# jeff-regier/Celeste.jl

Hardware: AMD Instinct MI355X
Metric: sources/sec (ELBO value+gradient+Hessian+KL per target source) (higher is better)
Workload: dtype f64; 1 GPU; BASELINE.json configs[2]: synthetic 2048x1489x5 SDSS-size field, 2000 star+galaxy sources, fp64, Sa=1 with value-only neighbours, psf_K=2; gather_backend=none, neighbor_links_rank0=3526

## Files before the change

celeste.jl_amd/csrc/celeste_abi.hip:

```cpp
#include <hip/hip_runtime.h>
#include <algorithm>
#include <atomic>
#include <cmath>
#include <cstdio>
#include <cstdlib>
#include <cstring>
#include <mutex>
#include <unordered_map>
#include <vector>

#include "elbo_kernels.h"
#include "optim_kernels.h"
#include "fused_kernels.h"
#include "host_tables.h"
#include "value_union.h"

struct celeste_group;

#define EVAL_FUSED_MAX 32

#define HIP_TRY(expr)                                                                    \
    do {                                                                                 \
        hipError_t e__ = (expr);                                                         \
        if (e__ != hipSuccess) {                                                         \
// ... 941 lines not shown
    HIP_TRY(hipGetLastError());
    return CELESTE_OK;
}

struct celeste_targets {
    celeste_ctx_t *ctx = nullptr;
    int32_t n = 0;
    int G = 1;
    int32_t *d_targets = nullptr;
    int32_t *d_work = nullptr, *d_work_total = nullptr, *d_rec_off = nullptr;
    int2 *d_items = nullptr;
    int32_t *d_needed = nullptr;
    int32_t *d_visits = nullptr;
    int32_t *d_vitems = nullptr;
    int4 *d_uitems = nullptr;
    int32_t *d_upx = nullptr;
    int64_t n_visits = 0, n_vitems = 0, n_uitems = 0;
    int64_t n_records = 0;
    int32_t n_work = 0;
    WorkSeqDesc *d_desc = nullptr;
    int32_t n_desc = 0;
};
static const int32_t LIST_STAMP = 1;

static void targets_free(celeste_targets *t) {
    if (!t) return;
    void *ptrs[] = {t->d_targets, t->d_work, t->d_work_total, t->d_rec_off, t->d_items, t->d_needed, t->d_visits, t->d_vitems,
                    t->d_uitems, t->d_upx, t->d_desc};
    for (void *p : ptrs) if (p) (void)hipFree(p);
    delete t;
}
// ... 6 lines not shown
    t->ctx = c; t->n = n; t->G = chunk_group(n);
    int32_t *d_blk = nullptr;
    auto fail = [&](int st) { if (d_blk) (void)hipFree(d_blk); (void)hipGetLastError(); targets_free(t); return st; };
#define LIST_TRY(expr) do { if ((expr) != hipSuccess) return fail(CELESTE_ERR_HIP); } while (0)
#define LIST_ALLOC(p, bytes) do { if (hipMalloc((void **)&(p), (bytes)) != hipSuccess) return fail(CELESTE_ERR_ALLOC); } while (0)
    std::vector<char> is_tgt((size_t)c->S, 0), reads((size_t)c->S, 0);
    for (int32_t s : tg) {
        is_tgt[s] = 1; reads[s] = 1;
        for (int64_t q = c->h_nbr_off[s]; q < c->h_nbr_off[s + 1]; ++q) reads[c->h_nbr_idx[q]] = 1;
        t->n_records += c->h_src_chunks[s];
    }
    std::vector<int32_t> visits, vitems;
    for (int s = 0; s < c->S; ++s)
        if (reads[s]) for (int v = c->h_vis_off[s]; v < c->h_vis_off[s + 1]; ++v) visits.push_back(v);
    for (size_t i = 0; i < c->h_vitem_tgt.size(); ++i) if (is_tgt[c->h_vitem_tgt[i]]) vitems.push_back((int32_t)i);
    std::vector<int32_t> upx;
    std::vector<ValueUnionItem> uitems;
    {
        static_assert(sizeof(ValueUnionBox) == 4 * sizeof(int32_t) && sizeof(ValueUnionItem) == sizeof(int4), "layout");
        std::vector<ValueUnionBox> boxes(c->h_patches.size());
        for (size_t v = 0; v < boxes.size(); ++v) { const DevPatch &q = c->h_patches[v]; boxes[v] = {q.off_h, q.off_w, q.H2, q.W2}; }
        std::vector<ValueUnionLink> links;
        links.reserve(vitems.size());
        for (int32_t i : vitems) links.push_back(c->h_vitem_link[(size_t)i]);
        if (!value_union_build(boxes.data(), std::move(links), c->chunk_px, upx, uitems)) return fail(CELESTE_ERR_INVALID_ARG);
    }
    t->n_visits = (int64_t)visits.size(); t->n_vitems = (int64_t)vitems.size(); t->n_uitems = (int64_t)uitems.size();
    const int n_cand = n * c->M;
    const int n_wblk = (n_cand + WORK_NT - 1) / WORK_NT;
    const size_t n_blk = (size_t)n_wblk * (WORK_CLASSES + 1);
    LIST_ALLOC(t->d_targets, (size_t)n * sizeof(int32_t));
    LIST_ALLOC(t->d_work, std::max<size_t>((size_t)t->n_records, 1) * sizeof(int32_t));
    LIST_ALLOC(t->d_work_total, sizeof(int32_t));
    LIST_ALLOC(t->d_rec_off, (size_t)n_cand * sizeof(int32_t));
    if (!c->dense) LIST_ALLOC(t->d_items, (size_t)n_cand * sizeof(int2));
    LIST_ALLOC(t->d_needed, (size_t)c->S * sizeof(int32_t));
    LIST_ALLOC(t->d_visits, std::max<size_t>(visits.size(), 1) * sizeof(int32_t));
    LIST_ALLOC(t->d_vitems, std::max<size_t>(vitems.size(), 1) * sizeof(int32_t));
    LIST_ALLOC(t->d_uitems, std::max<size_t>(uitems.size(), 1) * sizeof(int4));
    LIST_ALLOC(t->d_upx, std::max<size_t>(upx.size(), 1) * sizeof(int32_t));
    LIST_ALLOC(d_blk, n_blk * sizeof(int32_t));
    LIST_TRY(hipMemcpy(t->d_targets, tg.data(), (size_t)n * sizeof(int32_t), hipMemcpyHostToDevice));
    if (!visits.empty()) LIST_TRY(hipMemcpy(t->d_visits, visits.data(), visits.size() * sizeof(int32_t), hipMemcpyHostToDevice));
    if (!vitems.empty()) LIST_TRY(hipMemcpy(t->d_vitems, vitems.data(), vitems.size() * sizeof(int32_t), hipMemcpyHostToDevice));
    if (!uitems.empty()) LIST_TRY(hipMemcpy(t->d_uitems, uitems.data(), uitems.size() * sizeof(int4), hipMemcpyHostToDevice));
    if (!upx.empty()) LIST_TRY(hipMemcpy(t->d_upx, upx.data(), upx.size() * sizeof(int32_t), hipMemcpyHostToDevice));
    LIST_TRY(hipMemset(t->d_needed, 0, (size_t)c->S * sizeof(int32_t)));
    const size_t setup_threads = (size_t)n * (c->dense ? 1 : c->M);
    hipLaunchKernelGGL(setup_kernel, dim3((unsigned)((setup_threads + 63) / 64)), dim3(64), 0, nullptr, (const double *)nullptr, -1,
                       (SrcGeo *)nullptr, t->d_targets, n, c->d_vis_off, c->d_vis_img, c->M, t->d_items, t->d_needed, LIST_STAMP,
                       (int32_t *)nullptr, c->d_nbr_off, c->d_nbr_idx, (const int32_t *)nullptr);
    hipLaunchKernelGGL(work_count_kernel, dim3(n_wblk), dim3(WORK_NT), 0, nullptr, t->d_targets, n_cand, c->d_patches,
                       c->d_vis_off, c->d_vis_img, c->N, c->M, c->chunk_px, t->G, (int)c->dense, d_blk, (const int32_t *)nullptr);
    hipLaunchKernelGGL(work_scan_kernel, dim3(1), dim3(1024), 0, nullptr, d_blk, (int)n_blk, t->d_work_total, n_wblk * WORK_CLASSES);
    hipLaunchKernelGGL(work_fill_kernel, dim3(n_wblk), dim3(WORK_NT), 0, nullptr, t->d_targets, n_cand, c->d_patches,
                       c->d_vis_off, c->d_vis_img, c->N, c->M, c->CH, c->chunk_px, t->G, (int)c->dense, d_blk, t->d_work,
                       (const int32_t *)nullptr, t->d_rec_off);
    LIST_TRY(hipGetLastError());
    LIST_TRY(hipMemcpy(&t->n_work, t->d_work_total, sizeof(int32_t), hipMemcpyDeviceToHost));
    LIST_TRY(hipFree(d_blk)); d_blk = nullptr;
    if (t->n_work < 0 || (int64_t)t->n_work > t->n_records) return fail(CELESTE_ERR_HIP);
// ... 85 lines not shown
    if (need > c->acc_cap) {
        if (c->d_acc) { HIP_TRY(hipStreamSynchronize(stream)); HIP_TRY(hipFree(c->d_acc)); c->d_acc = nullptr; }
        HIP_TRY(hipMalloc((void **)&c->d_acc, need * sizeof(double)));
        c->acc_cap = need;
    }
    const int CH = c->CH, chunk_px = c->chunk_px;
    if (c->timing) HIP_TRY(hipEventRecord(c->ev[0], stream));
    const unsigned geo_blocks = (unsigned)((c->S + 63) / 64);
    hipLaunchKernelGGL(geo_prep_kernel, dim3(geo_blocks + (unsigned)t->n_visits), dim3(64), 0, stream, d_vp, c->d_images,
                       c->d_patches, c->d_vis_src, c->d_vis_img, c->K, c->d_srcimg, c->d_comps, t->d_visits, (int)geo_blocks,
                       c->S, c->d_geo);
    const char *no_union = getenv("CELESTE_NO_VALUE_UNION");
    if (!(no_union && atoi(no_union) != 0)) {
        if (t->n_uitems > 0) {
            const bool wide_items = n_targets <= VALUE_WIDE_MAX && c->chunk_px == 256 && !getenv("CELESTE_NO_WIDE_VALUE");
#define LAUNCH_UNION(WAVES)                                                                                                 \
            hipLaunchKernelGGL((value_union_kernel<WAVES>), dim3((unsigned)t->n_uitems), dim3(64 * WAVES), 0, stream,       \
                               c->d_patches, c->d_coefs, c->d_srcimg, c->d_comps, c->d_val_off, t->d_uitems, t->d_upx,      \
                               c->NC, c->d_val)
            if (wide_items) LAUNCH_UNION(4); else LAUNCH_UNION(1);
#undef LAUNCH_UNION
        }
    } else if (t->n_vitems > 0) {
        const bool wide_items = n_targets <= VALUE_WIDE_MAX && c->chunk_px == 256 && !getenv("CELESTE_NO_WIDE_VALUE");
#define LAUNCH_VALUE(WAVES)                                                                                                 \
        hipLaunchKernelGGL((value_kernel<double, WAVES>), dim3((unsigned)t->n_vitems), dim3(64 * WAVES), 0, stream,        \
                           c->d_patches, c->d_coefs, c->d_srcimg, c->d_comps, t->d_needed, LIST_STAMP, c->d_val_off,        \
                           c->d_value_items, c->NC, c->chunk_px, c->d_val, c->d_coefs_f, t->d_vitems)
        if (wide_items) LAUNCH_VALUE(4); else LAUNCH_VALUE(1);
#undef LAUNCH_VALUE
    }
    if (c->timing) HIP_TRY(hipEventRecord(c->ev[1], stream));
    const char *no_seq = getenv("CELESTE_NO_SEQUENCES");
    const bool sequences = !(no_seq && atoi(no_seq) != 0);
    const dim3 grid((unsigned)std::max<int32_t>(sequences ? t->n_desc : t->n_work, 1));
// ... 1086 lines not shown
```

celeste.jl_amd/csrc/elbo_kernels.h:

```cpp
#pragma once
#include <hip/hip_runtime.h>
#include <math.h>
#include "elbo_device.h"
#include "work_sequences.h"
#include "../../include/celeste_mi355x.h"

#ifndef CELESTE_MUTANT
#define CELESTE_MUTANT 0
#endif

__constant__ double c_eta[16];
__constant__ double c_nu[16];

__device__ inline void bvn_cov(double ab, double angle, double scale, double &x11, double &x12, double &x22) {
    double sp, cp;
    sincos(angle, &sp, &cp);
    double ab_term = ab * ab - 1.0;
    double s2 = scale * scale;
    x12 = -s2 * cp * sp * ab_term;
    x11 = s2 * (1.0 + ab_term * (sp * sp));
    x22 = s2 * (1.0 + ab_term * (cp * cp));
}

__device__ inline void brightness(const double *vs, int i, int b, double &El, double &Ell) {
// ... 323 lines not shown
#endif
    p = __builtin_fma(p, r, 1.6666666666666666e-01);
    p = __builtin_fma(p, r, 0.5);
    p = __builtin_fma(p, r, 1.0);
    return __builtin_fma(p, r, 1.0);
}
__device__ __forceinline__ double exp_nonpos(double x, const double *tab) {
    const double n = rint(x * EXP_INV_STEP);
    double r = __builtin_fma(n, -EXP_STEP_HI, x);
    r = __builtin_fma(n, EXP_STEP_LO, r);
    const int ni = (int)n;
    const double tj = tab[ni & (EXP_T - 1)];
    return ldexp(exp_poly(r) * tj, ni >> EXP_TAB_LOG2);
}

__device__ __forceinline__ double rcp_pos(double b) {
    double r = __builtin_amdgcn_rcp(b);
    r = __builtin_fma(__builtin_fma(-b, r, 1.0), r, r);
    return __builtin_fma(__builtin_fma(-b, r, 1.0), r, r);
}
__device__ __forceinline__ double log_pos(double x) {
    const bool ok = x > 2.2250738585072014e-308 && x < INFINITY;
    const double bad = x == INFINITY ? x : __builtin_nan("");
    double m = __builtin_amdgcn_frexp_mant(x);
    int e = __builtin_amdgcn_frexp_exp(x);
    const bool low = m < 0.7071067811865476;
    m = low ? m + m : m; e = low ? e - 1 : e;
    const double a = m - 1.0, b = m + 1.0, r = rcp_pos(b);
    double sq = a * r;
    sq = __builtin_fma(__builtin_fma(-b, sq, a), r, sq);
    const double z = sq * sq;
    double p = 1.0 / 21.0;
    p = __builtin_fma(p, z, 1.0 / 19.0); p = __builtin_fma(p, z, 1.0 / 17.0); p = __builtin_fma(p, z, 1.0 / 15.0);
    p = __builtin_fma(p, z, 1.0 / 13.0); p = __builtin_fma(p, z, 1.0 / 11.0); p = __builtin_fma(p, z, 1.0 / 9.0);
    p = __builtin_fma(p, z, 1.0 / 7.0); p = __builtin_fma(p, z, 1.0 / 5.0); p = __builtin_fma(p, z, 1.0 / 3.0);
    const double t = sq * z * p, ef = (double)e;
    const double lg = __builtin_fma(ef, 0x1.62e42fee00000p-1, (sq + sq) + __builtin_fma(ef, 0x1.a39ef35793c76p-33, t + t));
    return ok ? lg : bad;
}

__device__ inline double star_value(const double *__restrict__ coef, double xh, double xw) {
    int ix = (int)floor(xh); ix = ix < 1 ? 1 : (ix > 50 ? 50 : ix);
    int iy = (int)floor(xw); iy = iy < 1 ? 1 : (iy > 50 ? 50 : iy);
    double wx[4], wy[4];
    bspline_w(xh - ix, wx); bspline_w(xw - iy, wy);
    const double *c0 = coef + (ix - 1) + CEL_COEF * (iy - 1);
    double y = 0;
#pragma unroll
    for (int b = 0; b < 4; ++b) {
        const double *cb = c0 + CEL_COEF * b;
        double r = cb[0] * wx[0] + cb[1] * wx[1] + cb[2] * wx[2] + cb[3] * wx[3];
        y += r * wy[b];
    }
    return y < 0 ? 1e-3 * exp(y) : 1e-3 * (y + 1.0);
}

__device__ inline double galaxy_value(const Comp *tc, int NC, double dx, double dy, const double *etab) {
    double v = 0;
    const int n_dev = 8 * (NC / 14);
    for (int c0 = 0; c0 < NC; c0 += (c0 < n_dev ? 8 : 6)) {
        const int len = c0 < n_dev ? 8 : 6;
        const double d1 = dx - tc[c0].xi1, d2 = dy - tc[c0].xi2;
        const double s11 = -0.5 * (d1 * d1), s12 = -(d1 * d2), s22 = -0.5 * (d2 * d2);
        for (int c = c0; c < c0 + len; ++c) {
            const Comp k = tc[c];
            v = __builtin_fma(k.w0, exp_nonpos(__builtin_fma(k.p11, s11, __builtin_fma(k.p12, s12, k.p22 * s22)), etab), v);
        }
    }
    return v;
}

__device__ inline float star_value_f(const double *__restrict__ coef, float xh, float xw) {
    int ix = (int)floorf(xh); ix = ix < 1 ? 1 : (ix > 50 ? 50 : ix);
    int iy = (int)floorf(xw); iy = iy < 1 ? 1 : (iy > 50 ? 50 : iy);
    float wx[4], wy[4];
    bspline_w(xh - (float)ix, wx); bspline_w(xw - (float)iy, wy);
    const double *c0 = coef + (ix - 1) + CEL_COEF * (iy - 1);
    float y = 0;
#pragma unroll
    for (int b = 0; b < 4; ++b) {
        const double *cb = c0 + CEL_COEF * b;
        const float r = (float)cb[0] * wx[0] + (float)cb[1] * wx[1] + (float)cb[2] * wx[2] + (float)cb[3] * wx[3];
        y += r * wy[b];
// ... 347 lines not shown
            int first;
            const int n_rec = describe_target_records(ti, targets[ti], patches, nullptr, N, M, fz_chunk_px, rec_off, fz_chunk_desc, first);
            fz_tgt_rec[ti] = make_int2(first < 0 ? 0 : first, n_rec);
        }
    }
}

template <bool COH, typename R = double>
__device__ __forceinline__ void value_pixel(const DevPatch &P, const SrcImg &si, const Comp *__restrict__ tc, int NC,
                                            const double *__restrict__ coef, const double *__restrict__ etab, double sh0,
                                            double sw0, int h0, int w0, double2 *__restrict__ out,
                                            const float *__restrict__ tcf = nullptr) {
    const double hh = (double)(h0 + 1), ww = (double)(w0 + 1);
    double f0, f1;
    if constexpr (sizeof(R) == 8) {
        f0 = star_value(coef, hh + sh0, ww + sw0);
        f1 = galaxy_value(tc, NC, hh - si.m1, ww - si.m2, etab);
    } else {
        f0 = (double)star_value_f(coef, (float)(hh + sh0), (float)(ww + sw0));
        f1 = (double)galaxy_value_f(tcf, NC, (float)(hh - si.m1), (float)(ww - si.m2));
    }
    const double En = si.c0 * f0 + si.c1 * f1;
    const double E2n = si.q0 * (f0 * f0) + si.q1 * (f1 * f1);
    double2 *const o = out + ((h0 - P.off_h) + (int64_t)P.H2 * (w0 - P.off_w));
    const double var = E2n - En * En;
    if constexpr (COH) { stc<true>(&o->x, En); stc<true>(&o->y, var); }
    else *o = make_double2(En, var);
}

template <bool COH, typename R = double>
__device__ __forceinline__ void value_pixels(int lane, const DevPatch &P, const SrcImg &si, const Comp *__restrict__ tc, int NC,
// ... 149 lines not shown
        value_pixels<false, R>(threadIdx.x, P, si, tc, NC, coefs, etab, h_lo, w_lo, RH, p0, p1, val + val_off[sn], tcf);
    else {
        const int q0 = p0 + 64 * (int)(threadIdx.x >> 6);
        if (q0 < p1) value_pixels<false, R>(threadIdx.x & 63, P, si, tc, NC, coefs, etab, h_lo, w_lo, RH, q0, min(p1, q0 + 64), val + val_off[sn], tcf);
    }
    VT(2);
#ifdef VALUE_TIMING
    if (threadIdx.x == 0) {
        for (int k = 0; k < 3; ++k) atomicAdd(&g_value_clk[k], (unsigned long long)(vts[k + 1] - vts[k]));
        atomicAdd(&g_value_clk[7], 1ull); atomicAdd(&g_value_clk[6], (unsigned long long)((p1 - p0 + 63) / 64));
    }
#endif
#undef VT
}

template <int WAVES = 1>
__global__ void __launch_bounds__(64 * WAVES)
value_union_kernel(const DevPatch *__restrict__ patches, const double *__restrict__ coefs,
                   const SrcImg *__restrict__ srcimg, const Comp *__restrict__ comps, const int64_t *__restrict__ val_off,
                   const int4 *__restrict__ items, const int32_t *__restrict__ px_off, int NC, double2 *__restrict__ val) {
    __shared__ double etab[64];
    const int4 it = items[blockIdx.x];
    const int sn = it.x, count = it.z;
    const int32_t *__restrict__ po = px_off + it.y;
    const int lane = threadIdx.x & 63;
    int o0 = 0, o1 = 0, o2 = 0, o3 = 0;
    if constexpr (WAVES == 1) {
        if (lane < count) o0 = po[lane];
        if (lane + 64 < count) o1 = po[lane + 64];
        if (lane + 128 < count) o2 = po[lane + 128];
        if (lane + 192 < count) o3 = po[lane + 192];
    } else if ((int)threadIdx.x < count) o0 = po[threadIdx.x];
    const DevPatch &P = patches[sn];
    exp_table_init(etab);
    const SrcImg si = srcimg[sn];
    __shared__ Comp tc[14 * CEL_MAXK];
    {
        const double *src = reinterpret_cast<const double *>(comps + (size_t)sn * NC);
        double *dst = reinterpret_cast<double *>(tc);
        for (int i = threadIdx.x; i < NC * 8; i += 64 * WAVES) dst[i] = src[i];
        __syncthreads();
    }
    const double *__restrict__ coef = coefs + (size_t)(CELESTE_MUTANT == 3 ? 0 : P.stamp) * (CEL_COEF * CEL_COEF);
    const double sh0 = 26.0 - si.m1, sw0 = 26.0 - si.m2;
    const int H2 = P.H2;
    const float rH2 = 1.0f / (float)H2;
    double2 *__restrict__ out = val + val_off[sn];
    if constexpr (WAVES == 1) {
        for (int base = 0;;) {
            const int n = min(count - base, 256);
            for (int p = lane; p < n; p += 64) {
                int cw, ch;
                divmod_small(o0, H2, rH2, cw, ch);
                o0 = o1; o1 = o2; o2 = o3;
                value_pixel<false, double>(P, si, tc, NC, coef, etab, sh0, sw0, P.off_h + ch, P.off_w + cw, out);
            }
            base += 256;
            if (base >= count) break;
            const int i = base + lane;
            o0 = i < count ? po[i] : 0; o1 = i + 64 < count ? po[i + 64] : 0;
            o2 = i + 128 < count ? po[i + 128] : 0; o3 = i + 192 < count ? po[i + 192] : 0;
        }
    } else if ((int)threadIdx.x < count) {
        int cw, ch;
        divmod_small(o0, H2, rH2, cw, ch);
        value_pixel<false, double>(P, si, tc, NC, coef, etab, sh0, sw0, P.off_h + ch, P.off_w + cw, out);
    }
}

template <typename S>
struct PixelTermsT {
    typedef S scalar;
    S vterm, cnt_act, cnt_inact;
    S f0, f1;
    S alpha, beta, w2, w12;
    S k0, k1;
    S f0g0, f0g1, f0h0, f0h1, f0h2;
    S C0s, C0g, C1s, C1g;
    S Q0s, Q0g, Q1s, Q1g;
    S Wgg, Wsg, Wss;
    S S0d, S1x, S1y, S1xd, S1yd, S2a, S2b, S2c, S2an, S2bn, S2cn, S2ad, S2bd, S2cd;
    S S3a, S3b, S3c, S3d, S4a, S4b, S4c, S4d, S4e;
// ... 487 lines not shown
        const bool in_range = base + lane < p1;
        int w2, h2;
        divmod_small(idx, H2, 1.0f / (float)H2, w2, h2);
        const int h = P.off_h + h2 + 1, w = P.off_w + w2 + 1;
        const double hh = (double)h, ww = (double)w;
#define LOAD_PIXEL_INPUTS() load_pixel_inputs<MULTI, COHV>(img, P, W.patches, W.bitmaps, W.nbr_idx, W.nv, W.nb0, W.nb1, W.val_off, \
                                                     W.val, W.active_rank, W.my_rank, W.N, W.n, H2, h, w, h2, w2, in_range)
        const bool own_geo = in_range && (w2 < W2 - 1);
        if (MODE == 0) {
            const PixelInputs I = LOAD_PIXEL_INPUTS();
            const bool valid = I.valid, dup = I.dup, own = valid && own_geo;
            const double x = I.x, Ebar = I.Ebar, Vbar = I.Vbar, lgx = I.lgx, iota = I.iota, log_iota = I.log_iota;
            const int n_inact = I.n_inact;
            double f0 = 0, f1 = 0;
            if (own) {
                f0 = star_value(tcoef, hh + sh0, ww + sw0);
                f1 = galaxy_value(W.tc, NC, hh - si.m1, ww - si.m2, etab);
            }
            if (valid) {
                const double c0 = si.c0, c1 = si.c1, q0 = si.q0, q1 = si.q1;
                const double A = c0 * f0 + c1 * f1;
                const double E = Ebar + A;
                const double V = Vbar + ((q0 * (f0 * f0) + q1 * (f1 * f1)) - A * A);
                const double iE = 1.0 / E;
                if (!(MULTI && dup)) a[0] += x * (log_iota + (log(E) - V * (0.5 * iE * iE))) - iota * E - lgx;
                a[1] += own ? 1.0 : 0.0;
                a[2] += (double)n_inact;
            }
            return;
        }

// ... 1381 lines not shown
    const SrcImg si = srcimg[sn];
    __shared__ Comp tc[14 * CEL_MAXK];
    {
        const double *src = reinterpret_cast<const double *>(comps + (size_t)sn * NC);
        double *dst = reinterpret_cast<double *>(tc);
        for (int i = threadIdx.x; i < NC * 8; i += 64) dst[i] = src[i];
        __syncthreads();
    }
    const double *__restrict__ coef = coefs + (size_t)(CELESTE_MUTANT == 3 ? 0 : P.stamp) * (CEL_COEF * CEL_COEF);
    for (int idx = p0 + (int)threadIdx.x; idx < p1; idx += 64) {
        const int w2 = idx / H2, h2 = idx - w2 * H2;
        const size_t gi = (size_t)(P.off_h + h2) + (size_t)imgH * (P.off_w + w2);
        bool act = P.bitmap_off >= 0 ? bitmaps[P.bitmap_off + h2 + (int64_t)H2 * w2] != 0 : !isnan(pixels[gi]);
        if (!act) continue;
        const double hh = (double)(P.off_h + h2 + 1), ww = (double)(P.off_w + w2 + 1);
        const double f0 = star_value(coef, hh + (26.0 - si.m1), ww + (26.0 - si.m2));
        const double f1 = galaxy_value(tc, NC, hh - si.m1, ww - si.m2, etab);
        atomicAdd(&plane[gi], si.c0 * f0 + si.c1 * f1);
    }
}

__global__ void psf_raster_kernel(const double *__restrict__ psf, int K, const double *__restrict__ rows, int nr,
                                  const double *__restrict__ cols, int nc, double *__restrict__ out) {
    const int idx = blockIdx.x * blockDim.x + threadIdx.x;
    if (idx >= nr * nc) return;
    const int c = idx / nr, r = idx - c * nr;
    double s = 0;
    for (int k = 0; k < K; ++k) {
        const double *pc = psf + 6 * k;
        const double x0 = rows[r] - pc[1], x1 = cols[c] - pc[2];
        const double det = pc[3] * pc[5] - pc[4] * pc[4];
// ... 7 lines not shown
```

celeste.jl_amd/csrc/fit/celeste_fit.hip:

```cpp
#include "../celeste_abi.hip"
#include "../../../include/celeste_fit.h"

#define FIT_NB CELESTE_FIT_BANDS
#define FIT_NS CELESTE_FIT_NSTATS
#define FIT_REC 8

struct FitItem {
    int32_t sn, n;
    int32_t p0;
    int32_t rec0;
    int64_t stamp_off;
};

struct FitTileInfo { int32_t n_pix, bad, band, pad; };

__device__ __forceinline__ double fit_light(const SrcImg &si, const Comp *tc, int NC, const double *__restrict__ coef,
                                            const double *etab, double hh, double ww) {
    const double f0 = star_value(coef, hh + (26.0 - si.m1), ww + (26.0 - si.m2));
    const double f1 = galaxy_value(tc, NC, hh - si.m1, ww - si.m2, etab);
    return si.c0 * f0 + si.c1 * f1;
}

__device__ __forceinline__ double fit_wave_max(double x) {
#pragma unroll
    for (int o = 32; o >= 1; o >>= 1) x = fmax(x, __shfl_xor(x, o, 64));
    return x;
}

__device__ __forceinline__ void fit_stage_comps(Comp *dst, const Comp *__restrict__ src, int NC) {
    const double *s = reinterpret_cast<const double *>(src);
    double *d = reinterpret_cast<double *>(dst);
    for (int i = threadIdx.x; i < NC * 8; i += 64) d[i] = s[i];
}
// ... 268 lines not shown
```

celeste.jl_amd/csrc/mcmc/celeste_mcmc.hip:

```cpp
#include <hip/hip_runtime.h>
#include <algorithm>
#include <cmath>
#include <cstdio>
#include <cstring>
#include <mutex>
#include <new>
#include <vector>

#include "../elbo_kernels.h"
#include "../host_tables.h"
#include "../../../include/celeste_mcmc.h"

#define MC_D CELESTE_MCMC_D
#define MC_STEP_OUT 10
#define MC_ACCEPT_MAX 1000
#define MC_SHRINK_DEFAULT 10000

struct U4 { uint32_t x[4]; };
__host__ __device__ inline U4 philox4x32_10(U4 c, uint32_t k0, uint32_t k1) {
    for (int r = 0; r < 10; ++r) {
        if (r) { k0 += 0x9E3779B9u; k1 += 0xBB67AE85u; }
        const uint64_t p0 = (uint64_t)0xD2511F53u * c.x[0], p1 = (uint64_t)0xCD9E8D57u * c.x[2];
        U4 o;
        o.x[0] = (uint32_t)(p1 >> 32) ^ c.x[1] ^ k0;
// ... 80 lines not shown
    const double *coef = A.coefs + (size_t)P.stamp * (CEL_COEF * CEL_COEF);
    for (int64_t e = A.nbr_off[src]; e < A.nbr_off[src + 1]; ++e) {
        const celeste_mcmc_source_t &n = A.sources[A.nbr_idx[e]];
        double vs[6] = {n.pos[0], n.pos[1], n.gal_frac_dev, n.gal_axis_ratio, n.gal_angle, n.gal_radius_px};
        double m1, m2;
        world_to_pix(vs, P, m1, m2);
        const bool star = n.is_star != 0;
        const double flux = star ? n.star_fluxes[b] : n.gal_fluxes[b];
        __syncthreads();
        if (!star) prep_visit_values<false>(lane, vs, P, b, A.K, nullptr, tc);
        __syncthreads();
        const double sh0 = 26.0 - m1, sw0 = 26.0 - m2;
        for (int idx = lane; idx < npx; idx += 64) {
            const int w2 = idx / P.H2, h2 = idx - w2 * P.H2;
            const double hh = (double)(P.off_h + h2 + 1), ww = (double)(P.off_w + w2 + 1);
            const double f = star ? star_value(coef, hh + sh0, ww + sw0) : galaxy_value(tc, A.NC, hh - m1, ww - m2, etab);
            A.bgf[po + idx] = (float)((double)A.bgf[po + idx] + f * flux);
        }
    }
    for (int idx = lane; idx < npx; idx += 64) A.bg[po + idx] = (double)A.bgf[po + idx];
}

__device__ inline void mc_position(const double *box, const double *th, double &ra, double &dec) {
    ra = (box[1] - box[0]) * th[5] + box[0];
    dec = (box[3] - box[2]) * th[6] + box[2];
}

__device__ double mc_loglike(const McArgs &A, int ti, int model, const double *th, Comp *tc, const double *etab, int lane) {
    double ra, dec;
    mc_position(A.box + 4 * ti, th, ra, dec);
    double vs[6] = {ra, dec, 0.0, 0.0, 0.0, 0.0};
// ... 7 lines not shown
        const double flux = exp(th[b]);
        if (isinf(flux)) return -INFINITY;
        double m1, m2;
        world_to_pix(vs, P, m1, m2);
        if (model == 1) {
            __syncthreads();
            prep_visit_values<false>(lane, vs, P, b, A.K, nullptr, tc);
            __syncthreads();
        }
        const double *coef = A.coefs + (size_t)P.stamp * (CEL_COEF * CEL_COEF);
        const double sh0 = 26.0 - m1, sw0 = 26.0 - m2;
        const int64_t po = A.mv_pix[v];
        for (int idx = lane; idx < npx; idx += 64) {
            const int w2 = idx / P.H2, h2 = idx - w2 * P.H2;
            const double hh = (double)(P.off_h + h2 + 1), ww = (double)(P.off_w + w2 + 1);
            const double f = model == 0 ? star_value(coef, hh + sh0, ww + sw0) : galaxy_value(tc, A.NC, hh - m1, ww - m2, etab);
            const float srcf = (float)(f * flux);
            const double rate = ((double)srcf + A.bg[po + idx]) * (double)img.iota[P.off_h + h2];
            inf |= isinf(rate);
            const double x = A.data[po + idx];
            if (!isnan(x)) acc += x * log(rate) - rate;
        }
        lgs += A.lg[v];
    }
    if (__any(inf)) return -INFINITY;
    return wave_sum(acc) - lgs;
}

__device__ inline double mc_logsumexp8(const double *x) {
    double m = x[0];
    for (int k = 1; k < 8; ++k) m = fmax(m, x[k]);
// ... 613 lines not shown
```

celeste.jl_amd/csrc/synth/celeste_synth.hip:

```cpp
#include <hip/hip_runtime.h>
#include <algorithm>
#include <cmath>
#include <cstring>
#include <mutex>
#include <vector>

#include "../elbo_kernels.h"
#include "../host_tables.h"
#include "../../../include/celeste_synth.h"
#include "synth_sampler.h"

#define SYN_TH 64
#define SYN_TW 32
#define SYN_WAVES 4
#define SYN_COLS (SYN_TW / SYN_WAVES)
#define SYN_CHUNK 64
#define SYN_NCMAX (14 * CELESTE_SYNTH_MAX_K)

struct SynImage {
    int32_t H, W, K;
    uint32_t stream;
    const float *sky;
    const float *iota;
    double *lam;
// ... 70 lines not shown
            if (stamp < 0) {
                __syncthreads();
                const double *src = reinterpret_cast<const double *>(A.tables + (size_t)ent[e].table * SYN_NCMAX);
                for (int k = threadIdx.x; k < NC * (int)(sizeof(Comp) / sizeof(double)); k += 256) reinterpret_cast<double *>(tc)[k] = src[k];
                __syncthreads();
            }
            const int h0 = ent[e].h0, h1 = ent[e].h1, w0 = ent[e].w0, w1 = ent[e].w1;
            const double m1 = ent[e].m1, m2 = ent[e].m2, flux = ent[e].flux;
            const double *coef = A.coefs + (size_t)(stamp < 0 ? 0 : stamp) * (CEL_COEF * CEL_COEF);
            if (row_ok && h >= h0 && h <= h1) {
#pragma unroll
                for (int j = 0; j < SYN_COLS; ++j) {
                    const int w = T.w_start + wv + SYN_WAVES * j + 1;
                    if (w < w0 || w > w1) continue;
                    const double ww = (double)w;
                    const double f = stamp >= 0 ? star_value(coef, hh - m1 + 26.0, ww - m2 + 26.0)
                                                : galaxy_value(tc, NC, hh - m1, ww - m2, etab);
                    acc[j] += f * flux;
                }
            }
        }
    }
    if (!row_ok) return;
    const double iota = (double)img.iota[h - 1];
    unsigned long long ncap = 0;
    for (int j = 0; j < SYN_COLS; ++j) {
        const int w = T.w_start + wv + SYN_WAVES * j + 1;
        if (w > img.W) continue;
        const size_t q = (size_t)(h - 1) + (size_t)img.H * (w - 1);
        const double lam = acc[j] * iota;
        if (img.lam) img.lam[q] = lam;
// ... 259 lines not shown
```

celeste.jl_amd/csrc/value_union.h:

```cpp
#pragma once
#include <algorithm>
#include <cstddef>
#include <cstdint>
#include <vector>

struct ValueUnionBox { int32_t off_h, off_w, H2, W2; };
struct ValueUnionLink { int32_t vb, va; };
struct ValueUnionItem { int32_t vb, first, count, trips; };

inline bool value_union_build(const ValueUnionBox *boxes, std::vector<ValueUnionLink> links, int chunk_px,
                              std::vector<int32_t> &offsets, std::vector<ValueUnionItem> &items) {
    offsets.clear(); items.clear();
    std::sort(links.begin(), links.end(), [](const ValueUnionLink &a, const ValueUnionLink &b) {
        return a.vb != b.vb ? a.vb < b.vb : a.va < b.va;
    });
    links.erase(std::unique(links.begin(), links.end(), [](const ValueUnionLink &a, const ValueUnionLink &b) {
        return a.vb == b.vb && a.va == b.va;
    }), links.end());
    const int n_cls = chunk_px / 64;
    std::vector<std::vector<ValueUnionItem>> by_len((size_t)std::max(n_cls, 1));
    std::vector<unsigned char> wanted;
    for (size_t i = 0; i < links.size();) {
        const int32_t vb = links[i].vb;
        const ValueUnionBox &b = boxes[vb];
        const size_t npx = b.H2 > 0 && b.W2 > 0 ? (size_t)b.H2 * (size_t)b.W2 : 0;
        wanted.assign(npx, 0);
        for (; i < links.size() && links[i].vb == vb; ++i) {
            const ValueUnionBox &a = boxes[links[i].va];
            const int64_t h_lo = std::max(a.off_h, b.off_h), h_hi = std::min((int64_t)a.off_h + a.H2, (int64_t)b.off_h + b.H2);
            const int64_t w_lo = std::max(a.off_w, b.off_w), w_hi = std::min((int64_t)a.off_w + a.W2, (int64_t)b.off_w + b.W2 - 1);
            for (int64_t w = w_lo; w < w_hi; ++w)
                for (int64_t h = h_lo; h < h_hi; ++h) wanted[(size_t)((h - b.off_h) + (int64_t)b.H2 * (w - b.off_w))] = 1;
        }
        const size_t first = offsets.size();
        for (size_t p = 0; p < npx; ++p) if (wanted[p]) offsets.push_back((int32_t)p);
        const size_t count = offsets.size() - first;
        if (offsets.size() > (size_t)INT32_MAX) { offsets.clear(); items.clear(); return false; }
        for (size_t p0 = 0; p0 < count; p0 += (size_t)chunk_px) {
            const int32_t px = (int32_t)std::min((size_t)chunk_px, count - p0), trips = (px + 63) / 64;
            by_len[(size_t)(n_cls - trips)].push_back({vb, (int32_t)(first + p0), px, trips});
        }
    }
    for (auto &v : by_len) items.insert(items.end(), v.begin(), v.end());
    return true;
}
```

Before: 3.243 million sources/sec.

## Precompute packed (h,w) offsets, hoist star spline weights, cheaper exp in value path

The value-union builder now emits pixel offsets packed as 16-bit row/column pairs, so the kernel no longer needs a per-pixel divmod. When every lane's sub-cell fraction matches the first pixel, the kernel hoists the star B-spline weights into wave-uniform scalars, and falls back to the old path otherwise. Galaxy exp evaluation pre-scales its arguments by the inverse step and uses an unnormalised polynomial with one final rescale. The star softplus uses a table-based degree-5 exp. These changes cut VALU work in the value-only neighbour pass, at the cost of small numeric differences and a new wave ballot per pixel.

```diff
diff --git a/celeste.jl_amd/csrc/celeste_abi.hip b/celeste.jl_amd/csrc/celeste_abi.hip
--- a/celeste.jl_amd/csrc/celeste_abi.hip
+++ b/celeste.jl_amd/csrc/celeste_abi.hip
@@ -979,7 +979,7 @@
     int32_t *d_visits = nullptr;
     int32_t *d_vitems = nullptr;
     int4 *d_uitems = nullptr;
-    int32_t *d_upx = nullptr;
+    uint32_t *d_upx = nullptr;
     int64_t n_visits = 0, n_vitems = 0, n_uitems = 0;
     int64_t n_records = 0;
     int32_t n_work = 0;
@@ -1016,7 +1016,8 @@
     for (int s = 0; s < c->S; ++s)
         if (reads[s]) for (int v = c->h_vis_off[s]; v < c->h_vis_off[s + 1]; ++v) visits.push_back(v);
     for (size_t i = 0; i < c->h_vitem_tgt.size(); ++i) if (is_tgt[c->h_vitem_tgt[i]]) vitems.push_back((int32_t)i);
-    std::vector<int32_t> upx;
+    std::vector<int32_t> uoff;
+    std::vector<uint32_t> upx;
     std::vector<ValueUnionItem> uitems;
     {
         static_assert(sizeof(ValueUnionBox) == 4 * sizeof(int32_t) && sizeof(ValueUnionItem) == sizeof(int4), "layout");
@@ -1025,7 +1026,7 @@
         std::vector<ValueUnionLink> links;
         links.reserve(vitems.size());
         for (int32_t i : vitems) links.push_back(c->h_vitem_link[(size_t)i]);
-        if (!value_union_build(boxes.data(), std::move(links), c->chunk_px, upx, uitems)) return fail(CELESTE_ERR_INVALID_ARG);
+        if (!value_union_build(boxes.data(), std::move(links), c->chunk_px, uoff, uitems, &upx)) return fail(CELESTE_ERR_INVALID_ARG);
     }
     t->n_visits = (int64_t)visits.size(); t->n_vitems = (int64_t)vitems.size(); t->n_uitems = (int64_t)uitems.size();
     const int n_cand = n * c->M;
@@ -1040,13 +1041,13 @@
     LIST_ALLOC(t->d_visits, std::max<size_t>(visits.size(), 1) * sizeof(int32_t));
     LIST_ALLOC(t->d_vitems, std::max<size_t>(vitems.size(), 1) * sizeof(int32_t));
     LIST_ALLOC(t->d_uitems, std::max<size_t>(uitems.size(), 1) * sizeof(int4));
-    LIST_ALLOC(t->d_upx, std::max<size_t>(upx.size(), 1) * sizeof(int32_t));
+    LIST_ALLOC(t->d_upx, std::max<size_t>(upx.size(), 1) * sizeof(uint32_t));
     LIST_ALLOC(d_blk, n_blk * sizeof(int32_t));
     LIST_TRY(hipMemcpy(t->d_targets, tg.data(), (size_t)n * sizeof(int32_t), hipMemcpyHostToDevice));
     if (!visits.empty()) LIST_TRY(hipMemcpy(t->d_visits, visits.data(), visits.size() * sizeof(int32_t), hipMemcpyHostToDevice));
     if (!vitems.empty()) LIST_TRY(hipMemcpy(t->d_vitems, vitems.data(), vitems.size() * sizeof(int32_t), hipMemcpyHostToDevice));
     if (!uitems.empty()) LIST_TRY(hipMemcpy(t->d_uitems, uitems.data(), uitems.size() * sizeof(int4), hipMemcpyHostToDevice));
-    if (!upx.empty()) LIST_TRY(hipMemcpy(t->d_upx, upx.data(), upx.size() * sizeof(int32_t), hipMemcpyHostToDevice));
+    if (!upx.empty()) LIST_TRY(hipMemcpy(t->d_upx, upx.data(), upx.size() * sizeof(uint32_t), hipMemcpyHostToDevice));
     LIST_TRY(hipMemset(t->d_needed, 0, (size_t)c->S * sizeof(int32_t)));
     const size_t setup_threads = (size_t)n * (c->dense ? 1 : c->M);
     hipLaunchKernelGGL(setup_kernel, dim3((unsigned)((setup_threads + 63) / 64)), dim3(64), 0, nullptr, (const double *)nullptr, -1,
@@ -1162,11 +1163,15 @@
     if (!(no_union && atoi(no_union) != 0)) {
         if (t->n_uitems > 0) {
             const bool wide_items = n_targets <= VALUE_WIDE_MAX && c->chunk_px == 256 && !getenv("CELESTE_NO_WIDE_VALUE");
-#define LAUNCH_UNION(WAVES)                                                                                                 \
-            hipLaunchKernelGGL((value_union_kernel<WAVES>), dim3((unsigned)t->n_uitems), dim3(64 * WAVES), 0, stream,       \
+            const char *no_hoist = getenv("CELESTE_NO_VALUE_HOIST");
+            const bool hoist = !(no_hoist && atoi(no_hoist) != 0);
+#define LAUNCH_UNION(WAVES, HOIST)                                                                                          \
+            hipLaunchKernelGGL((value_union_kernel<WAVES, HOIST>), dim3((unsigned)t->n_uitems), dim3(64 * WAVES), 0, stream,\
                                c->d_patches, c->d_coefs, c->d_srcimg, c->d_comps, c->d_val_off, t->d_uitems, t->d_upx,      \
                                c->NC, c->d_val)
-            if (wide_items) LAUNCH_UNION(4); else LAUNCH_UNION(1);
+            if (wide_items) { if (hoist) LAUNCH_UNION(4, true); else LAUNCH_UNION(4, false); }
+            else if (hoist) LAUNCH_UNION(1, true);
+            else LAUNCH_UNION(1, false);
 #undef LAUNCH_UNION
         }
     } else if (t->n_vitems > 0) {
diff --git a/celeste.jl_amd/csrc/elbo_kernels.h b/celeste.jl_amd/csrc/elbo_kernels.h
--- a/celeste.jl_amd/csrc/elbo_kernels.h
+++ b/celeste.jl_amd/csrc/elbo_kernels.h
@@ -361,6 +361,47 @@
     return ldexp(exp_poly(r) * tj, ni >> EXP_TAB_LOG2);
 }
 
+#ifndef CELESTE_VALUE_DIET
+#define CELESTE_VALUE_DIET 1
+#endif
+#if EXP_DEGREE == 4
+#define EXP_STEPS_SCALE (EXP_STEP_FULL * EXP_STEP_FULL * EXP_STEP_FULL * EXP_STEP_FULL)
+#else
+#define EXP_STEPS_SCALE 1.0
+#endif
+__device__ __forceinline__ double scalar_reg(double c) { asm("" : "+s"(c)); return c; }
+__device__ __forceinline__ double exp_steps_nonpos(double y, const double *tab) {
+    const double n = rint(y);
+    const double r = y - n;
+    const int ni = (int)n;
+    const double tj = tab[ni & (EXP_T - 1)];
+    double p;
+#if EXP_DEGREE == 4
+    p = r + 4.0 / EXP_STEP_FULL;
+    p = __builtin_fma(p, r, scalar_reg(12.0 / (EXP_STEP_FULL * EXP_STEP_FULL)));
+    p = __builtin_fma(p, r, scalar_reg(24.0 / (EXP_STEP_FULL * EXP_STEP_FULL * EXP_STEP_FULL)));
+    p = __builtin_fma(p, r, scalar_reg(24.0 / (EXP_STEP_FULL * EXP_STEP_FULL * EXP_STEP_FULL * EXP_STEP_FULL)));
+#else
+    p = exp_poly(r * EXP_STEP_FULL);
+#endif
+    return ldexp(p * tj, ni >> EXP_TAB_LOG2);
+}
+__device__ __forceinline__ double exp_nonpos_d5(double x, const double *tab) {
+    const double n = rint(x * EXP_INV_STEP);
+    double r = __builtin_fma(n, -EXP_STEP_HI, x);
+    r = __builtin_fma(n, EXP_STEP_LO, r);
+    const int ni = (int)n;
+    const double tj = tab[ni & (EXP_T - 1)];
+    constexpr double U = EXP_DEGREE == 4 ? 24.0 : 1.0;
+    double p = U / 120.0;
+    p = __builtin_fma(p, r, U / 24.0);
+    p = __builtin_fma(p, r, U / 6.0);
+    p = __builtin_fma(p, r, U * 0.5);
+    p = __builtin_fma(p, r, U);
+    p = __builtin_fma(p, r, U);
+    return ldexp(p * tj, ni >> EXP_TAB_LOG2);
+}
+
 __device__ __forceinline__ double rcp_pos(double b) {
     double r = __builtin_amdgcn_rcp(b);
     r = __builtin_fma(__builtin_fma(-b, r, 1.0), r, r);
@@ -386,12 +427,11 @@
     return ok ? lg : bad;
 }
 
-__device__ inline double star_value(const double *__restrict__ coef, double xh, double xw) {
-    int ix = (int)floor(xh); ix = ix < 1 ? 1 : (ix > 50 ? 50 : ix);
-    int iy = (int)floor(xw); iy = iy < 1 ? 1 : (iy > 50 ? 50 : iy);
-    double wx[4], wy[4];
-    bspline_w(xh - ix, wx); bspline_w(xw - iy, wy);
-    const double *c0 = coef + (ix - 1) + CEL_COEF * (iy - 1);
+__device__ __forceinline__ void star_cell(double x, int &i, double &f) {
+    i = (int)floor(x); i = i < 1 ? 1 : (i > 50 ? 50 : i);
+    f = x - i;
+}
+__device__ __forceinline__ double star_spline(const double *__restrict__ c0, const double (&wx)[4], const double (&wy)[4]) {
     double y = 0;
 #pragma unroll
     for (int b = 0; b < 4; ++b) {
@@ -399,21 +439,54 @@
         double r = cb[0] * wx[0] + cb[1] * wx[1] + cb[2] * wx[2] + cb[3] * wx[3];
         y += r * wy[b];
     }
+    return y;
+}
+__device__ __forceinline__ double star_softplus(double y, const double *etab) {
+#if CELESTE_VALUE_DIET
+    return y < 0 ? 1e-3 * exp_nonpos_d5(y, etab) : 1e-3 * (y + 1.0);
+#else
+    (void)etab;
     return y < 0 ? 1e-3 * exp(y) : 1e-3 * (y + 1.0);
-}
-
+#endif
+}
+__device__ inline double star_value(const double *__restrict__ coef, double xh, double xw, const double *etab) {
+    int ix, iy;
+    double fx, fy, wx[4], wy[4];
+    star_cell(xh, ix, fx); star_cell(xw, iy, fy);
+    bspline_w(fx, wx); bspline_w(fy, wy);
+    return star_softplus(star_spline(coef + (ix - 1) + CEL_COEF * (iy - 1), wx, wy), etab);
+}
+
+template <int LEN>
+__device__ __forceinline__ double galaxy_value_run(const Comp *tr, double s11, double s12, double s22, const double *etab, double v) {
+#pragma unroll
+    for (int c = 0; c < LEN; ++c) {
+        const double x = __builtin_fma(tr[c].p11, s11, __builtin_fma(tr[c].p12, s12, tr[c].p22 * s22));
+#if CELESTE_VALUE_DIET
+        v = __builtin_fma(tr[c].w0, exp_steps_nonpos(x, etab), v);
+#else
+        v = __builtin_fma(tr[c].w0, exp_nonpos(x, etab), v);
+#endif
+    }
+    return v;
+}
 __device__ inline double galaxy_value(const Comp *tc, int NC, double dx, double dy, const double *etab) {
     double v = 0;
     const int n_dev = 8 * (NC / 14);
     for (int c0 = 0; c0 < NC; c0 += (c0 < n_dev ? 8 : 6)) {
         const int len = c0 < n_dev ? 8 : 6;
         const double d1 = dx - tc[c0].xi1, d2 = dy - tc[c0].xi2;
+#if CELESTE_VALUE_DIET
+        const double s11 = (-0.5 * EXP_INV_STEP) * (d1 * d1), s12 = -EXP_INV_STEP * (d1 * d2), s22 = (-0.5 * EXP_INV_STEP) * (d2 * d2);
+#else
         const double s11 = -0.5 * (d1 * d1), s12 = -(d1 * d2), s22 = -0.5 * (d2 * d2);
-        for (int c = c0; c < c0 + len; ++c) {
-            const Comp k = tc[c];
-            v = __builtin_fma(k.w0, exp_nonpos(__builtin_fma(k.p11, s11, __builtin_fma(k.p12, s12, k.p22 * s22)), etab), v);
-        }
-    }
+#endif
+        v = galaxy_value_run<6>(tc + c0, s11, s12, s22, etab, v);
+        if (len == 8) v = galaxy_value_run<2>(tc + c0 + 6, s11, s12, s22, etab, v);
+    }
+#if CELESTE_VALUE_DIET
+    v *= EXP_STEPS_SCALE;
+#endif
     return v;
 }
 
@@ -791,7 +864,7 @@
     const double hh = (double)(h0 + 1), ww = (double)(w0 + 1);
     double f0, f1;
     if constexpr (sizeof(R) == 8) {
-        f0 = star_value(coef, hh + sh0, ww + sw0);
+        f0 = star_value(coef, hh + sh0, ww + sw0, etab);
         f1 = galaxy_value(tc, NC, hh - si.m1, ww - si.m2, etab);
     } else {
         f0 = (double)star_value_f(coef, (float)(hh + sh0), (float)(ww + sw0));
@@ -971,17 +1044,23 @@
 #undef VT
 }
 
-template <int WAVES = 1>
+#ifndef VALUE_UNION_SPLIT_BITS
+#define VALUE_UNION_SPLIT_BITS 16
+#endif
+__device__ __forceinline__ double uniform_double(double x) {
+    return __hiloint2double(__builtin_amdgcn_readfirstlane(__double2hiint(x)), __builtin_amdgcn_readfirstlane(__double2loint(x)));
+}
+template <int WAVES = 1, bool HOIST = true>
 __global__ void __launch_bounds__(64 * WAVES)
 value_union_kernel(const DevPatch *__restrict__ patches, const double *__restrict__ coefs,
                    const SrcImg *__restrict__ srcimg, const Comp *__restrict__ comps, const int64_t *__restrict__ val_off,
-                   const int4 *__restrict__ items, const int32_t *__restrict__ px_off, int NC, double2 *__restrict__ val) {
+                   const int4 *__restrict__ items, const uint32_t *__restrict__ px, int NC, double2 *__restrict__ val) {
     __shared__ double etab[64];
     const int4 it = items[blockIdx.x];
     const int sn = it.x, count = it.z;
-    const int32_t *__restrict__ po = px_off + it.y;
+    const uint32_t *__restrict__ po = px + it.y;
     const int lane = threadIdx.x & 63;
-    int o0 = 0, o1 = 0, o2 = 0, o3 = 0;
+    uint32_t o0 = 0, o1 = 0, o2 = 0, o3 = 0;
     if constexpr (WAVES == 1) {
         if (lane < count) o0 = po[lane];
         if (lane + 64 < count) o1 = po[lane + 64];
@@ -1001,16 +1080,45 @@
     const double *__restrict__ coef = coefs + (size_t)(CELESTE_MUTANT == 3 ? 0 : P.stamp) * (CEL_COEF * CEL_COEF);
     const double sh0 = 26.0 - si.m1, sw0 = 26.0 - si.m2;
     const int H2 = P.H2;
-    const float rH2 = 1.0f / (float)H2;
     double2 *__restrict__ out = val + val_off[sn];
+    constexpr uint32_t CMASK = (1u << VALUE_UNION_SPLIT_BITS) - 1;
+    auto plain = [&](uint32_t q) {
+        int ch = (int)(q & CMASK), cw = (int)(q >> VALUE_UNION_SPLIT_BITS);
+        if constexpr (!HOIST) divmod_small(ch + H2 * cw, H2, 1.0f / (float)H2, cw, ch);
+        value_pixel<false, double>(P, si, tc, NC, coef, etab, sh0, sw0, P.off_h + ch, P.off_w + cw, out);
+    };
     if constexpr (WAVES == 1) {
+        double fx0 = 0, fy0 = 0, wx0[4] = {0, 0, 0, 0}, wy0[4] = {0, 0, 0, 0};
+        if constexpr (HOIST) {
+            const uint32_t q = po[0];
+            int i0;
+            star_cell((double)(P.off_h + (int)(q & CMASK) + 1) + sh0, i0, fx0);
+            star_cell((double)(P.off_w + (int)(q >> VALUE_UNION_SPLIT_BITS) + 1) + sw0, i0, fy0);
+            bspline_w(fx0, wx0); bspline_w(fy0, wy0);
+            fx0 = uniform_double(fx0); fy0 = uniform_double(fy0);
+#pragma unroll
+            for (int b = 0; b < 4; ++b) { wx0[b] = uniform_double(wx0[b]); wy0[b] = uniform_double(wy0[b]); }
+        }
         for (int base = 0;;) {
             const int n = min(count - base, 256);
             for (int p = lane; p < n; p += 64) {
-                int cw, ch;
-                divmod_small(o0, H2, rH2, cw, ch);
+                const uint32_t q = o0;
                 o0 = o1; o1 = o2; o2 = o3;
-                value_pixel<false, double>(P, si, tc, NC, coef, etab, sh0, sw0, P.off_h + ch, P.off_w + cw, out);
+                if constexpr (HOIST) {
+                    const int ch = (int)(q & CMASK), cw = (int)(q >> VALUE_UNION_SPLIT_BITS);
+                    const double hh = (double)(P.off_h + ch + 1), ww = (double)(P.off_w + cw + 1);
+                    int ix, iy;
+                    double fx, fy;
+                    star_cell(hh + sh0, ix, fx); star_cell(ww + sw0, iy, fy);
+                    if (__builtin_amdgcn_ballot_w64(fx != fx0 || fy != fy0) != 0) { plain(q); continue; }
+                    const double y = star_spline(coef + (ix - 1) + CEL_COEF * (iy - 1), wx0, wy0);
+                    const double f0 = star_softplus(y, etab);
+                    const double f1 = galaxy_value(tc, NC, hh - si.m1, ww - si.m2, etab);
+                    const double En = si.c0 * f0 + si.c1 * f1;
+                    const double E2n = si.q0 * (f0 * f0) + si.q1 * (f1 * f1);
+                    const double var = E2n - En * En;
+                    out[(uint32_t)(ch + H2 * cw)] = make_double2(En, var);
+                } else plain(q);
             }
             base += 256;
             if (base >= count) break;
@@ -1018,11 +1126,7 @@
             o0 = i < count ? po[i] : 0; o1 = i + 64 < count ? po[i + 64] : 0;
             o2 = i + 128 < count ? po[i + 128] : 0; o3 = i + 192 < count ? po[i + 192] : 0;
         }
-    } else if ((int)threadIdx.x < count) {
-        int cw, ch;
-        divmod_small(o0, H2, rH2, cw, ch);
-        value_pixel<false, double>(P, si, tc, NC, coef, etab, sh0, sw0, P.off_h + ch, P.off_w + cw, out);
-    }
+    } else if ((int)threadIdx.x < count) plain(o0);
 }
 
 template <typename S>
@@ -1540,7 +1644,7 @@
             const int n_inact = I.n_inact;
             double f0 = 0, f1 = 0;
             if (own) {
-                f0 = star_value(tcoef, hh + sh0, ww + sw0);
+                f0 = star_value(tcoef, hh + sh0, ww + sw0, etab);
                 f1 = galaxy_value(W.tc, NC, hh - si.m1, ww - si.m2, etab);
             }
             if (valid) {
@@ -2952,7 +3056,7 @@
         bool act = P.bitmap_off >= 0 ? bitmaps[P.bitmap_off + h2 + (int64_t)H2 * w2] != 0 : !isnan(pixels[gi]);
         if (!act) continue;
         const double hh = (double)(P.off_h + h2 + 1), ww = (double)(P.off_w + w2 + 1);
-        const double f0 = star_value(coef, hh + (26.0 - si.m1), ww + (26.0 - si.m2));
+        const double f0 = star_value(coef, hh + (26.0 - si.m1), ww + (26.0 - si.m2), etab);
         const double f1 = galaxy_value(tc, NC, hh - si.m1, ww - si.m2, etab);
         atomicAdd(&plane[gi], si.c0 * f0 + si.c1 * f1);
     }
diff --git a/celeste.jl_amd/csrc/fit/celeste_fit.hip b/celeste.jl_amd/csrc/fit/celeste_fit.hip
--- a/celeste.jl_amd/csrc/fit/celeste_fit.hip
+++ b/celeste.jl_amd/csrc/fit/celeste_fit.hip
@@ -16,7 +16,7 @@
 
 __device__ __forceinline__ double fit_light(const SrcImg &si, const Comp *tc, int NC, const double *__restrict__ coef,
                                             const double *etab, double hh, double ww) {
-    const double f0 = star_value(coef, hh + (26.0 - si.m1), ww + (26.0 - si.m2));
+    const double f0 = star_value(coef, hh + (26.0 - si.m1), ww + (26.0 - si.m2), etab);
     const double f1 = galaxy_value(tc, NC, hh - si.m1, ww - si.m2, etab);
     return si.c0 * f0 + si.c1 * f1;
 }
diff --git a/celeste.jl_amd/csrc/mcmc/celeste_mcmc.hip b/celeste.jl_amd/csrc/mcmc/celeste_mcmc.hip
--- a/celeste.jl_amd/csrc/mcmc/celeste_mcmc.hip
+++ b/celeste.jl_amd/csrc/mcmc/celeste_mcmc.hip
@@ -118,7 +118,7 @@
         for (int idx = lane; idx < npx; idx += 64) {
             const int w2 = idx / P.H2, h2 = idx - w2 * P.H2;
             const double hh = (double)(P.off_h + h2 + 1), ww = (double)(P.off_w + w2 + 1);
-            const double f = star ? star_value(coef, hh + sh0, ww + sw0) : galaxy_value(tc, A.NC, hh - m1, ww - m2, etab);
+            const double f = star ? star_value(coef, hh + sh0, ww + sw0, etab) : galaxy_value(tc, A.NC, hh - m1, ww - m2, etab);
             A.bgf[po + idx] = (float)((double)A.bgf[po + idx] + f * flux);
         }
     }
@@ -156,7 +156,7 @@
         for (int idx = lane; idx < npx; idx += 64) {
             const int w2 = idx / P.H2, h2 = idx - w2 * P.H2;
             const double hh = (double)(P.off_h + h2 + 1), ww = (double)(P.off_w + w2 + 1);
-            const double f = model == 0 ? star_value(coef, hh + sh0, ww + sw0) : galaxy_value(tc, A.NC, hh - m1, ww - m2, etab);
+            const double f = model == 0 ? star_value(coef, hh + sh0, ww + sw0, etab) : galaxy_value(tc, A.NC, hh - m1, ww - m2, etab);
             const float srcf = (float)(f * flux);
             const double rate = ((double)srcf + A.bg[po + idx]) * (double)img.iota[P.off_h + h2];
             inf |= isinf(rate);
diff --git a/celeste.jl_amd/csrc/synth/celeste_synth.hip b/celeste.jl_amd/csrc/synth/celeste_synth.hip
--- a/celeste.jl_amd/csrc/synth/celeste_synth.hip
+++ b/celeste.jl_amd/csrc/synth/celeste_synth.hip
@@ -108,7 +108,7 @@
                     const int w = T.w_start + wv + SYN_WAVES * j + 1;
                     if (w < w0 || w > w1) continue;
                     const double ww = (double)w;
-                    const double f = stamp >= 0 ? star_value(coef, hh - m1 + 26.0, ww - m2 + 26.0)
+                    const double f = stamp >= 0 ? star_value(coef, hh - m1 + 26.0, ww - m2 + 26.0, etab)
                                                 : galaxy_value(tc, NC, hh - m1, ww - m2, etab);
                     acc[j] += f * flux;
                 }
diff --git a/celeste.jl_amd/csrc/value_union.h b/celeste.jl_amd/csrc/value_union.h
--- a/celeste.jl_amd/csrc/value_union.h
+++ b/celeste.jl_amd/csrc/value_union.h
@@ -8,9 +8,16 @@
 struct ValueUnionLink { int32_t vb, va; };
 struct ValueUnionItem { int32_t vb, first, count, trips; };
 
+#ifndef VALUE_UNION_SPLIT_BITS
+#define VALUE_UNION_SPLIT_BITS 16
+#endif
+static_assert(VALUE_UNION_SPLIT_BITS == 16, "the kernel's unpacking (elbo_kernels.h) and the builder's packing");
 inline bool value_union_build(const ValueUnionBox *boxes, std::vector<ValueUnionLink> links, int chunk_px,
-                              std::vector<int32_t> &offsets, std::vector<ValueUnionItem> &items) {
+                              std::vector<int32_t> &offsets, std::vector<ValueUnionItem> &items,
+                              std::vector<uint32_t> *split = nullptr) {
     offsets.clear(); items.clear();
+    if (split) split->clear();
+    auto refuse = [&]() { offsets.clear(); items.clear(); if (split) split->clear(); return false; };
     std::sort(links.begin(), links.end(), [](const ValueUnionLink &a, const ValueUnionLink &b) {
         return a.vb != b.vb ? a.vb < b.vb : a.va < b.va;
     });
@@ -35,7 +42,16 @@
         const size_t first = offsets.size();
         for (size_t p = 0; p < npx; ++p) if (wanted[p]) offsets.push_back((int32_t)p);
         const size_t count = offsets.size() - first;
-        if (offsets.size() > (size_t)INT32_MAX) { offsets.clear(); items.clear(); return false; }
+        if (offsets.size() > (size_t)INT32_MAX) return refuse();
+        if (split) {
+            size_t p = 0;
+            for (int64_t cw = 0; cw < b.W2; ++cw)
+                for (int64_t ch = 0; ch < b.H2; ++ch, ++p)
+                    if (wanted[p]) {
+                        if ((ch | cw) >> VALUE_UNION_SPLIT_BITS) return refuse();
+                        split->push_back((uint32_t)ch | (uint32_t)cw << VALUE_UNION_SPLIT_BITS);
+                    }
+        }
         for (size_t p0 = 0; p0 < count; p0 += (size_t)chunk_px) {
             const int32_t px = (int32_t)std::min((size_t)chunk_px, count - p0), trips = (px + 63) / 64;
             by_len[(size_t)(n_cls - trips)].push_back({vb, (int32_t)(first + p0), px, trips});
```

After: 3.275 million sources/sec, median of 6. Within noise of the previous version (+1.0%).
